# ishine/Prior-DiffuSE

Measured on AMD Instinct MI355X. Metric: enhanced-audio sec/sec (RTF), 6-step fast sampling, B=32, higher is better.
Workload: dtype f16x2; 1 GPU; B=32 x 4 s 16 kHz utterances per GPU, [B,2,401,161] spectrograms, GCRN prior + DiffUNet1 6-step sampling, STFT..ISTFT, seeded random weights; global_batch=32, frames=401, parallelism=batch-shard x1, graph=True, streams_per_gpu=1, batches_in_flight=3

## Files before the change

### __graft_entry__.py

```python
import importlib
import os
import subprocess
import sys

ROOT = os.path.dirname(os.path.abspath(__file__))
PKG = os.path.join(ROOT, "prior-diffuse_amd")
CSRC = os.path.join(PKG, "csrc")
SOURCES = ["gconv.hip", "gconv2.hip", "gconv3.hip", "gconv4.hip", "misc.hip", "lstm.hip", "lstmp.hip", "aia.hip", "tcm.hip", "tcm2.hip", "bglu.hip", "gru3.hip", "dense.hip", "metrics.hip", "stoi.hip", "resample.hip", "wavout.hip", "range.hip", "valid.hip", "objective.hip", "ensemble.hip", "window.hip", "capi.hip"]
LIB = os.path.join(PKG, "libpdse.so")


HASHFILE = LIB + ".srchash"


def _source_hash():
    import hashlib

    h = hashlib.sha256()
    included = sorted(f for f in os.listdir(CSRC) if f.endswith((".h", ".inc")))
    deps = [os.path.join(CSRC, s) for s in SOURCES + included] + [os.path.join(ROOT, "include", "pdse.h")]
    for d in deps:
        with open(d, "rb") as f:
            h.update(os.path.basename(d).encode() + b"\0" + f.read())
    return h.hexdigest()


def _stale():
    if not (os.path.exists(LIB) and os.path.exists(HASHFILE)):
        return True
    with open(HASHFILE) as f:
        return f.read().strip() != _source_hash()


def build(force=False):
    import torch

    import fcntl

    with open(os.path.join(PKG, ".build.lock"), "w") as lock:
        fcntl.flock(lock, fcntl.LOCK_EX)
        if force or _stale():
# ... 65 lines not shown
```

### include/pdse.h

```cpp
#ifndef PDSE_H
#define PDSE_H
#include <stdint.h>

#ifdef __cplusplus
extern "C" {
#endif

#define PDSE_ABI_VERSION 9

typedef void* pdse_stream_t;

enum pdse_act { PDSE_ACT_NONE = 0, PDSE_ACT_PRELU = 1, PDSE_ACT_ELU = 2, PDSE_ACT_SIGMOID = 3 };

enum pdse_epi {
  PDSE_EPI_LINEAR = 0,
  PDSE_EPI_GLU = 1,
  PDSE_EPI_BIGLU = 2
};

typedef struct pdse_src {
  const float* ptr;
  int64_t sb, sc, st, sf;
  int32_t C;
  int32_t act;
// ... 27 lines not shown
  int32_t act;
  float act_slope;
  int32_t C2;
  const float* post_scale;
  const float* post_shift;
  const float* wlc;
  const float* wrc;
  const float* blc;
  const float* brc;
  const float* wc2;
  const float* bc2;
  const float* resid;
  float* out;
  int64_t out_sb, out_sc_hi, out_sc_lo, out_st, out_sf, out_off;
  int32_t out_cr;
  int32_t B, Tout, Fout;
  int32_t korder;
  int32_t ksteps1;
  const float* w2;
  const float* w3;
  int32_t p1mask;
  int32_t Fout1;
  const float* nx_w;
  const float* nx_bias[3];
  const float* nx_add[3];
  float* nx_out[3];
  int64_t nx_bias_sb[3];
  int64_t nx_sb[3], nx_sc[3], nx_st[3], nx_sf[3], nx_off[3];
  int32_t nx_n, nx_keep, nx_row0;
  int32_t wexp;
  const float* bias0_t0;
  const float* bias1_t0;
  int32_t tap_dt[12], tap_df[12];
  int32_t flat, pad_;
} pdse_gconv_desc;

typedef struct pdse_time_desc {
  const float* t;
  const float* table;
  const float* p1T;
  const float* b1;
  const float* p2T;
  const float* b2;
  const float* wfT;
  const float* bf;
  float* out;
  float* temb;
  int32_t B, NF, max_steps, pad_;
} pdse_time_desc;

enum pdse_ew_op {
  PDSE_EW_DIV = 0,
  PDSE_EW_UPDATE = 1,
  PDSE_EW_UPDATE_FINAL = 2,
  PDSE_EW_COPY = 3,
  PDSE_EW_ADD_MUL = 4
};
typedef struct pdse_ew_desc {
  const float* a;
  const float* b;
  const float* c;
  float* out;
  int64_t n;
  float s0, s1, s2;
  int32_t op;
} pdse_ew_desc;

// ... 634 lines not shown
```

### prior-diffuse_amd/_lib.py

```python
import contextlib
import ctypes as C
import os

_HERE = os.path.dirname(os.path.abspath(__file__))
LIB_PATH = os.environ.get("PDSE_LIB") or os.path.join(_HERE, "libpdse.so")

ABI_VERSION = 9

ACT_NONE, ACT_PRELU, ACT_ELU, ACT_SIGMOID = 0, 1, 2, 3
EPI_LINEAR, EPI_GLU, EPI_BIGLU = 0, 1, 2
EW_DIV, EW_UPDATE, EW_UPDATE_FINAL, EW_COPY, EW_ADD_MUL = 0, 1, 2, 3, 4
(OP_GCONV, OP_TIME, OP_EW, OP_COMPAND, OP_WAVPREP, OP_OLA, OP_SIGMA, OP_LN, OP_LSTM,
 OP_ROWLN, OP_CHLN, OP_ATTN, OP_GRU, OP_GNCOMB, OP_AHAM, OP_QSAMPLE, OP_TRANSPOSE, OP_TCM, OP_CRM, OP_GCRNLAST,
 OP_MASKLOSS, OP_GLSTM, OP_TCM2, OP_BGLU, OP_PLANES, OP_GLSTMP, OP_TCM2S, OP_DENSE, OP_ROWLNB, OP_METRICS, OP_RESAMPLE, OP_RANGE) = range(32)
MASKLOSS_BLOCKS = 32
SPECLOSS_BLOCKS = 32

ENSEMBLE_BLOCKS = 32
ENSEMBLE_MAX = 16
_fp = C.c_void_p
_i32, _i64, _f32 = C.c_int32, C.c_int64, C.c_float


class Src(C.Structure):
    _fields_ = [("ptr", _fp), ("sb", _i64), ("sc", _i64), ("st", _i64), ("sf", _i64),
                ("C", _i32), ("act", _i32), ("blk", _i32), ("pad_", _i32)]


class GconvDesc(C.Structure):
    _fields_ = [
        ("in0", Src), ("in1", Src),
        ("Tin", _i32), ("Fin", _i32),
        ("padrow", _fp), ("padrow_sb", _i64),
        ("taps", _fp), ("ntaps", _i32), ("sf_in", _i32),
        ("xf_scale0", _fp), ("xf_shift0", _fp), ("xf_scale1", _fp), ("xf_shift1", _fp),
        ("xf_slope0", _f32), ("xf_slope1", _f32), ("xf_mode", _i32), ("cin1", _i32),
        ("w0", _fp), ("w1", _fp), ("ksteps", _i32), ("Cout", _i32),
        ("bias0", _fp), ("bias1", _fp), ("bias0_sb", _i64), ("bias1_sb", _i64),
        ("epi", _i32), ("act", _i32), ("act_slope", _f32), ("C2", _i32),
        ("post_scale", _fp), ("post_shift", _fp),
        ("wlc", _fp), ("wrc", _fp), ("blc", _fp), ("brc", _fp), ("wc2", _fp), ("bc2", _fp),
        ("resid", _fp), ("out", _fp),
        ("out_sb", _i64), ("out_sc_hi", _i64), ("out_sc_lo", _i64), ("out_st", _i64),
        ("out_sf", _i64), ("out_off", _i64),
        ("out_cr", _i32), ("B", _i32), ("Tout", _i32), ("Fout", _i32),
        ("korder", _i32), ("ksteps1", _i32), ("w2", _fp), ("w3", _fp), ("p1mask", _i32), ("Fout1", _i32),
        ("nx_w", _fp), ("nx_bias", _fp * 3), ("nx_add", _fp * 3), ("nx_out", _fp * 3), ("nx_bias_sb", _i64 * 3),
        ("nx_sb", _i64 * 3), ("nx_sc", _i64 * 3), ("nx_st", _i64 * 3), ("nx_sf", _i64 * 3), ("nx_off", _i64 * 3),
        ("nx_n", _i32), ("nx_keep", _i32), ("nx_row0", _i32), ("wexp", _i32),
        ("bias0_t0", _fp), ("bias1_t0", _fp),
        ("tap_dt", _i32 * 12), ("tap_df", _i32 * 12), ("flat", _i32), ("pad_", _i32),
    ]


class TimeDesc(C.Structure):
    _fields_ = [("t", _fp), ("table", _fp), ("p1T", _fp), ("b1", _fp), ("p2T", _fp), ("b2", _fp),
                ("wfT", _fp), ("bf", _fp), ("out", _fp), ("temb", _fp),
                ("B", _i32), ("NF", _i32), ("max_steps", _i32), ("pad_", _i32)]


class EwDesc(C.Structure):
    _fields_ = [("a", _fp), ("b", _fp), ("c", _fp), ("out", _fp), ("n", _i64),
                ("s0", _f32), ("s1", _f32), ("s2", _f32), ("op", _i32)]


class CompandDesc(C.Structure):
    _fields_ = [("in_", _fp), ("out", _fp), ("plane", _i64), ("B", _i32), ("mode", _i32),
                ("out_sb", _i64), ("out_sc", _i64), ("out_st", _i64), ("F", _i32), ("pad_", _i32)]


COMPAND_SQRT, COMPAND_SQUARE, COMPAND_MAG, COMPAND_COPY, COMPAND_POW03, COMPAND_POW103, COMPAND_LOG1X, COMPAND_EXPM1 = range(8)
FEAT_TYPES = ("sqrt", "normal", "cubic", "log_1x", "none")
COMPRESS_MODE = {"sqrt": COMPAND_SQRT, "normal": COMPAND_MAG, "cubic": COMPAND_POW03, "log_1x": COMPAND_LOG1X, "none": None}
DECOMPRESS_MODE = {"sqrt": COMPAND_SQUARE, "normal": COMPAND_COPY, "cubic": COMPAND_POW103, "log_1x": COMPAND_EXPM1,
                   "none": COMPAND_COPY}


def feat_type_of(value):
    if value not in FEAT_TYPES:
        raise ValueError("feat_type %r: must be one of 'sqrt', 'normal', 'cubic', 'log_1x', 'none'" % (value,))
    return value


def members_arg(members):
# ... 521 lines not shown
```

### prior-diffuse_amd/csrc/capi.hip

```cpp
#include <hip/hip_runtime.h>
#include <stdint.h>
#include <stdio.h>
#include <string.h>

#include <new>
#include <string>
#include <vector>

#include "pdse.h"
#include "pdse_internal.h"

static thread_local std::string g_err;

void pdse_set_error(const char* msg) { g_err = msg ? msg : "unknown error"; }

int pdse_check_hip(hipError_t e, const char* what) {
  if (e == hipSuccess) return 0;
  g_err = std::string(what) + ": " + hipGetErrorString(e);
  return 1;
}

int pdse_check_launch(const char* what) { return pdse_check_hip(hipGetLastError(), what); }

int pdse_lds_attr(const void* fn, unsigned long long* mask, const char* what) {
// ... 45 lines not shown
  explicit device_guard(const pdse_plan* p) {
    if (!p || p->device < 0) return;
    if (hipGetDevice(&prev) != hipSuccess) prev = -1;
    if (prev != p->device) ok = !pdse_check_hip(hipSetDevice(p->device), "set device");
    else prev = -1;
  }
  ~device_guard() {
    if (prev >= 0) (void)hipSetDevice(prev);
  }
};

static int op_size(int kind) {
  switch (kind) {
#define X(KIND, stem, entry) case PDSE_OP_##KIND: return (int)sizeof(pdse_##stem##_desc);
    PDSE_OPS(X)
#undef X
    default: return -1;
  }
}

static int launch_op(const pdse_op& op, hipStream_t s) {
  switch (op.kind) {
#define X(KIND, stem, entry) case PDSE_OP_##KIND: return pdse_##stem##_launch(&op.d.stem, s);
    PDSE_OPS(X)
#undef X
    default: pdse_set_error("plan: unknown op kind"); return 1;
  }
}

static bool names_odd_phase(const pdse_op& op) {
  return op.kind == PDSE_OP_GCONV && op.d.gconv.korder == 5 && op.d.gconv.p1mask != 0 && op.d.gconv.w2 == nullptr;
}

static int check_follows(const pdse_plan* p, const pdse_op& op) {
  if (p->ops.empty() || !names_odd_phase(p->ops.back())) return 0;
  if (op.kind != PDSE_OP_GCONV) {
    pdse_set_error("plan: the operator behind a gconv that names its odd phase (p1mask, korder 5) must be that phase");
    return 1;
  }
  return pdse_gconv_pair_check(&p->ops.back().d.gconv, &op.d.gconv);
}

static int launch_at(const pdse_plan* p, const int i, const int end, hipStream_t s, int* n) {
  const pdse_op& op = p->ops[i];
  *n = 1;
  if (names_odd_phase(op) && i + 1 < end) {
    *n = 2;
    return pdse_gconv4_pair_launch(&op.d.gconv, &p->ops[i + 1].d.gconv, s);
  }
  return launch_op(op, s);
}

template <typename D>
static int validate_desc(const D*) { return 0; }
static int validate_desc(const pdse_range_desc* d) { return pdse_range_validate(d); }

extern "C" {

int pdse_abi_version(void) { return PDSE_ABI_VERSION; }
const char* pdse_last_error(void) { return g_err.c_str(); }
int pdse_desc_size(int op_kind) { return op_size(op_kind); }

#define X(KIND, stem, entry) \
  int entry(const pdse_##stem##_desc* d, pdse_stream_t s) { return validate_desc(d) ? 1 : pdse_##stem##_launch(d, (hipStream_t)s); }
PDSE_OPS(X)
#undef X

int pdse_wav_encode(const float* x, const int32_t* n_in_host, const int32_t* n_keep_host, const int32_t* n_in, const int32_t* n_keep,
                    const double* taps, uint8_t* out, int32_t* clipped, int64_t stride, int32_t B, int32_t Lmax, int32_t up, int32_t down,
                    int32_t half, int32_t fmt, int32_t width, int32_t ch, pdse_stream_t s) {
  return pdse_wavout_launch(x, n_in_host, n_keep_host, n_in, n_keep, taps, out, clipped, stride, B, Lmax, up, down, half, fmt, width, ch,
                            (hipStream_t)s);
}

int pdse_wav_encode_channels(const float* x, const int32_t* n_in_host, const int32_t* n_keep_host, const int32_t* n_in,
                             const int32_t* n_keep, const double* taps, uint8_t* out, int32_t* clipped, int64_t stride, int32_t B,
                             int32_t Lmax, int32_t up, int32_t down, int32_t half, int32_t fmt, int32_t width, int32_t ch, pdse_stream_t s) {
  return pdse_wavch_launch(x, n_in_host, n_keep_host, n_in, n_keep, taps, out, clipped, stride, B, Lmax, up, down, half, fmt, width, ch,
                           (hipStream_t)s);
}

// ... 441 lines not shown
```

### prior-diffuse_amd/csrc/gconv.hip

```cpp
#include <hip/hip_runtime.h>
#include <stdint.h>

#include "pdse.h"
#include "pdse_internal.h"

#include "gconv_common.h"

template <int EPI, int MT, bool CIN1>
__global__ __launch_bounds__(256) void gconv_kernel(const pdse_gconv_desc d) {
  constexpr bool DUAL = (EPI != PDSE_EPI_LINEAR);
  const int lane = threadIdx.x & 63, wave = threadIdx.x >> 6;
  const int col = lane & 31, h = lane >> 5;
  const int b = blockIdx.y;
  const int P = d.Tout * d.Fout;
  const int p = (blockIdx.x * 4 + wave) * 32 + col;
  const bool pvalid = p < P;
  const int t = pvalid ? p / d.Fout : 0;
  const int j = pvalid ? p - t * d.Fout : 0;
  const int mtiles = (d.Cout + 31) >> 5;
  const int mt0 = blockIdx.z * MT;

  f32x16 acc0[MT], acc1[DUAL ? MT : 1];
#pragma unroll
  for (int m = 0; m < MT; ++m) {
// ... 73 lines not shown
      float v = 0.f;
      if (pvalid && tap < d.ntaps) {
        const int tin = t + d.taps[2 * tap], fin = j * d.sf_in + d.taps[2 * tap + 1];
        if (tin >= 0 && tin < d.Tin && fin >= 0 && fin < d.Fin) {
          v = base[(int64_t)tin * S.st + (int64_t)fin * S.sf];
          if (S.act) v = act_f(v, S.act, 0.f);
        }
      }
#pragma unroll
      for (int m = 0; m < MT; ++m) {
        if (mt0 + m < mtiles) {
          const float a0 = wp0[((size_t)m * ksteps + ks) * 64];
          acc0[m] = __builtin_amdgcn_mfma_f32_32x32x2f32(a0, v, acc0[m], 0, 0, 0);
          if (DUAL) {
            const float a1 = wp1[((size_t)m * ksteps + ks) * 64];
            acc1[m] = __builtin_amdgcn_mfma_f32_32x32x2f32(a1, v, acc1[m], 0, 0, 0);
          }
        }
      }
    }
  }

  gconv_epilogue<EPI, MT>(d, tail_from_desc(d), acc0, acc1, b, t, j, pvalid, lane, h, mt0, mtiles);
}

#define PDSE_REQUIRE(cond, msg)    \
  do {                             \
    if (!(cond)) {                 \
      pdse_set_error("gconv: " msg); \
      return 1;                    \
    }                              \
  } while (0)

static int gconv_launch(const pdse_gconv_desc* d, hipStream_t s, const bool dry) {
  PDSE_REQUIRE(d != nullptr, "null descriptor");
  PDSE_REQUIRE(!dry || d->korder == 5, "a phase pair is two korder 5 launches");
  PDSE_REQUIRE(d->in0.ptr && d->out && d->w0 && d->taps, "null pointer (in0/out/w0/taps)");
  PDSE_REQUIRE(d->B > 0 && d->B <= 65535 && d->Tout > 0 && d->Fout > 0, "bad output extents");
  PDSE_REQUIRE(d->Cout > 0 && d->ntaps > 0 && d->out_cr > 0, "bad Cout/ntaps/out_cr");
  PDSE_REQUIRE((int64_t)d->Tout * d->Fout < (1ll << 30), "too many positions per batch item");
  const int Cin = d->in0.C + d->in1.C;
  if (d->cin1) {
    PDSE_REQUIRE(Cin == 1 && d->in1.C == 0, "cin1 path needs exactly one input channel");
    PDSE_REQUIRE(d->ksteps == (d->ntaps + 1) / 2, "ksteps != ceil(ntaps/2)");
    PDSE_REQUIRE(d->xf_mode == 0 && d->padrow == nullptr, "cin1 path has no load transform / pad row");
  } else {
    PDSE_REQUIRE(Cin >= 2 && (d->in0.C % 2) == 0 && (d->in1.C % 2) == 0, "channel counts must be even");
    PDSE_REQUIRE(d->in1.C == 0 || d->in1.ptr, "in1 has channels but no pointer");
    if (d->korder == 0) PDSE_REQUIRE(d->ksteps == d->ntaps * (Cin / 2), "ksteps != ntaps*Cin/2");
    else PDSE_REQUIRE(d->ksteps >= d->ntaps * (Cin / 2), "ksteps < ntaps*Cin/2");
    PDSE_REQUIRE(d->korder < 3 || d->epi != PDSE_EPI_BIGLU, "korder 3 / 4 / 5 have LINEAR / GLU epilogues only");
  }
  PDSE_REQUIRE((d->in0.blk == 0 && d->in1.blk == 0) || d->korder == 3 || d->korder == 4 || d->korder == 5, "channel-blocked sources (pdse_src.blk) are read by the korder 3 kernel only");
  PDSE_REQUIRE(d->flat == 0 || d->korder == 3 || d->korder == 5, "the flat form (pdse_gconv_desc.flat) is one of the korder 3 / 5 kernel");
  if (d->xf_mode) {
    PDSE_REQUIRE(d->xf_scale0 && d->xf_shift0, "xf_mode set without scale/shift");
    PDSE_REQUIRE(d->xf_mode != 2 || (d->xf_scale1 && d->xf_shift1), "xf_mode 2 without second set");
  }
  PDSE_REQUIRE((d->post_scale == nullptr) == (d->post_shift == nullptr), "post_scale/post_shift must come together");
  {
    auto al16 = [](const void* p) { return (reinterpret_cast<uintptr_t>(p) & 15) == 0; };
    PDSE_REQUIRE(al16(d->bias0) && al16(d->bias1) && al16(d->post_scale) && al16(d->post_shift) && al16(d->blc) &&
                     al16(d->brc) && al16(d->bc2) && al16(d->bias0_t0) && al16(d->bias1_t0),
                 "per-channel operands (biases, folded BatchNorm) must be 16-byte aligned");
    PDSE_REQUIRE((d->bias0_sb & 3) == 0 && (d->bias1_sb & 3) == 0, "bias batch strides must be multiples of 4 floats");
  }
  PDSE_REQUIRE(d->resid == nullptr || d->act == PDSE_ACT_NONE, "a residual input excludes an activation (x + f(..) is the last op)");
  if (d->nx_n != 0) {
    PDSE_REQUIRE(d->nx_n > 0 && d->nx_n <= 3 && d->nx_w, "nx: 1..3 chained tiles and their weights");
    PDSE_REQUIRE(d->epi == PDSE_EPI_BIGLU && (d->korder == 1 || d->korder == 2) && d->C2 == 64 && d->out_cr == 1,
                 "nx: chained 1x1 tiles need the pipelined BIGLU kernel with a 64-channel block output");
    for (int i = 0; i < d->nx_n; ++i) PDSE_REQUIRE(d->nx_bias[i] && d->nx_out[i], "nx: bias / output pointer missing");
    PDSE_REQUIRE(d->nx_row0 < d->nx_n, "nx_row0 out of range");
    PDSE_REQUIRE(d->w2 == nullptr || (d->nx_n == 1 && d->nx_keep == 0 && d->nx_row0 < 0),
                 "nx: a dual-phase launch chains one tile and does not keep its own output");
    PDSE_REQUIRE(d->nx_keep == 0 || d->out, "nx_keep without an output pointer");
  }
  PDSE_REQUIRE((d->bias0_t0 == nullptr) == (d->bias1_t0 == nullptr), "bias0_t0 / bias1_t0 must come together");
  PDSE_REQUIRE(d->bias0_t0 == nullptr || (d->nx_n > 0 && d->w2 == nullptr),
               "frame-0 biases are a feature of the chained single-phase BIGLU tail");
  if (d->korder == 1) {
    PDSE_REQUIRE(!d->cin1, "korder 1 needs Cin >= 2");
    return pdse_gconv2_launch(d, s);
  }
  if (d->korder >= 3 && d->korder <= 5) return dry ? 0 : pdse_gconv4_launch(d, s);
  if (d->korder == 2) {
    PDSE_REQUIRE(d->resid == nullptr, "BIGLU has no residual input");
    PDSE_REQUIRE(d->act == PDSE_ACT_NONE || d->act == PDSE_ACT_PRELU, "BIGLU stages end in PReLU or no activation");
    return pdse_gconv3_launch(d, s);
  }
  PDSE_REQUIRE(d->korder == 0, "unknown korder");
  const int mtiles = (d->Cout + 31) / 32;
  const int P = d->Tout * d->Fout;
  const int gx = ((P + 31) / 32 + 3) / 4;
  dim3 block(256);
  auto grid = [&](int mt) { return dim3(gx, d->B, (mtiles + mt - 1) / mt); };

#define LAUNCH(EPI, MT, C1)                                                          \
  hipLaunchKernelGGL((gconv_kernel<EPI, MT, C1>), grid(MT), block, 0, s, *d)

  switch (d->epi) {
    case PDSE_EPI_LINEAR: {
      if (d->cin1) {
        if (mtiles >= 4) LAUNCH(PDSE_EPI_LINEAR, 4, true);
        else if (mtiles >= 2) LAUNCH(PDSE_EPI_LINEAR, 2, true);
        else LAUNCH(PDSE_EPI_LINEAR, 1, true);
      } else {
        if (mtiles >= 4) LAUNCH(PDSE_EPI_LINEAR, 4, false);
        else if (mtiles >= 2) LAUNCH(PDSE_EPI_LINEAR, 2, false);
        else LAUNCH(PDSE_EPI_LINEAR, 1, false);
      }
      break;
    }
    case PDSE_EPI_GLU: {
      PDSE_REQUIRE(d->w1 != nullptr && !d->cin1, "GLU needs w1 and Cin >= 2");
      if (mtiles >= 4) LAUNCH(PDSE_EPI_GLU, 4, false);
      else if (mtiles >= 2) LAUNCH(PDSE_EPI_GLU, 2, false);
      else LAUNCH(PDSE_EPI_GLU, 1, false);
      break;
    }
    case PDSE_EPI_BIGLU: {
      PDSE_REQUIRE(d->w1 && !d->cin1 && d->Cout == 32, "BIGLU needs w1 and a 32-channel gate pair");
      PDSE_REQUIRE(d->bias0 && d->bias1 && d->wlc && d->wrc && d->blc && d->brc && d->wc2 && d->bc2,
                   "BIGLU chain pointers missing");
      PDSE_REQUIRE(d->C2 == 1 || (d->C2 > 0 && d->C2 % 32 == 0), "BIGLU C2 must be 1 or a multiple of 32");
      PDSE_REQUIRE(d->resid == nullptr, "BIGLU has no residual input");
      PDSE_REQUIRE(d->act == PDSE_ACT_NONE || d->act == PDSE_ACT_PRELU, "BIGLU stages end in PReLU or no activation");
      LAUNCH(PDSE_EPI_BIGLU, 1, false);
      break;
    }
    default:
      pdse_set_error("gconv: unknown epilogue");
      return 1;
  }
#undef LAUNCH
  return pdse_check_launch("gconv");
}

int pdse_gconv_launch(const pdse_gconv_desc* d, hipStream_t s) { return gconv_launch(d, s, false); }

int pdse_gconv_pair_check(const pdse_gconv_desc* d, const pdse_gconv_desc* e) {
  if (gconv_launch(d, nullptr, true) || gconv_launch(e, nullptr, true)) return 1;
  return pdse_gconv4_pair_check(d, e);
}
```

### prior-diffuse_amd/csrc/pdse_internal.h

```cpp
#ifndef PDSE_INTERNAL_H
#define PDSE_INTERNAL_H
#include <hip/hip_runtime.h>

#include "pdse.h"

void pdse_set_error(const char* msg);
int pdse_check_launch(const char* what);
int pdse_check_hip(hipError_t e, const char* what);
int pdse_lds_attr(const void* fn, unsigned long long* mask, const char* what);
#ifdef PDSE_DIAG
#define PDSE_DIAG_ENV(name) (getenv(name))
#else
#define PDSE_DIAG_ENV(name) ((const char*)nullptr)
#endif

#define PDSE_OPS(X)                                                                            \
  X(GCONV, gconv, pdse_gconv_f32)                                                              \
  X(TIME, time, pdse_time_embed_f32)                                                           \
  X(EW, ew, pdse_ew_f32)                                                                       \
  X(COMPAND, compand, pdse_compand_f32)                                                        \
  X(WAVPREP, wavprep, pdse_wavprep_f32)                                                        \
  X(OLA, ola, pdse_ola_f32)                                                                    \
  X(SIGMA, sigma, pdse_sigma_mask_f32)                                                         \
  X(LN, ln, pdse_layernorm_f32)                                                                \
// ... 1 lines not shown
  X(ROWLN, rowln, pdse_rowln_prelu_f32)                                                        \
  X(CHLN, chln, pdse_chln_f32)                                                                 \
  X(ATTN, attn, pdse_attention_f32)                                                            \
  X(GRU, gru, pdse_bigru_f32)                                                                  \
  X(GNCOMB, gncomb, pdse_gn_combine_f32)                                                       \
  X(AHAM, aham, pdse_aham_f32)                                                                 \
  X(QSAMPLE, qsample, pdse_qsample_f32)                                                        \
  X(TRANSPOSE, transpose, pdse_transpose_f32)                                                  \
  X(TCM, tcm, pdse_tcm_f32)                                                                    \
  X(CRM, crm, pdse_crm_f32)                                                                    \
  X(GCRNLAST, gcrnlast, pdse_gcrnlast_f32)                                                     \
  X(MASKLOSS, maskloss, pdse_masked_mse_f32)                                                   \
  X(GLSTM, glstm, pdse_glstm_f32)                                                              \
  X(TCM2, tcm2, pdse_tcm2_bf16x3)                                                              \
  X(BGLU, bglu, pdse_bglu_planes)                                                              \
  X(PLANES, planes, pdse_split_planes)                                                         \
  X(GLSTMP, glstmp, pdse_glstm_persistent_f32)                             \
  X(TCM2S, tcm2s, pdse_tcm2_stack_bf16x3)    \
  X(DENSE, dense, pdse_dense_layer_bf16x3)                                 \
  X(ROWLNB, rowlnb, pdse_rowln_blocked_f32)                                                    \
  X(METRICS, metrics, pdse_quality_metrics_f32)                          \
  X(RESAMPLE, resample, pdse_pcm_resample_f32)                          \
  X(RANGE, range, pdse_range_hist)

#define X(KIND, stem, entry) int pdse_##stem##_launch(const pdse_##stem##_desc* d, hipStream_t s);
PDSE_OPS(X)
#undef X
int pdse_gconv2_launch(const pdse_gconv_desc* d, hipStream_t s);
int pdse_gconv3_launch(const pdse_gconv_desc* d, hipStream_t s);
int pdse_gconv4_launch(const pdse_gconv_desc* d, hipStream_t s);
int pdse_gconv_pair_check(const pdse_gconv_desc* d, const pdse_gconv_desc* e);
int pdse_gconv4_pair_check(const pdse_gconv_desc* d, const pdse_gconv_desc* e);
int pdse_gconv4_pair_launch(const pdse_gconv_desc* d, const pdse_gconv_desc* e, hipStream_t s);
int pdse_stoi_launch(const pdse_metrics_desc* d, hipStream_t s);
int pdse_gru3_launch(const pdse_gru_desc* d, hipStream_t s);
int pdse_wavout_launch(const float* x, const int32_t* n_in_host, const int32_t* n_keep_host, const int32_t* n_in, const int32_t* n_keep,
                       const double* taps, uint8_t* out, int32_t* clipped, int64_t stride, int32_t B, int32_t Lmax, int32_t up,
                       int32_t down, int32_t half, int32_t fmt, int32_t width, int32_t ch, hipStream_t s);
int pdse_wavch_launch(const float* x, const int32_t* n_in_host, const int32_t* n_keep_host, const int32_t* n_in, const int32_t* n_keep,
                      const double* taps, uint8_t* out, int32_t* clipped, int64_t stride, int32_t B, int32_t Lmax, int32_t up,
                      int32_t down, int32_t half, int32_t fmt, int32_t width, int32_t ch, hipStream_t s);
int pdse_pair_prep_launch(const float* noisy, const float* clean, const int32_t* lens, float* noisy_pad, float* clean_pad, float* c,
                          int32_t B, int32_t L, int32_t pad, int32_t reflect_own, hipStream_t s);
int pdse_spec_losses_launch(const float* esti, const float* label, const int32_t* frames_host, const int32_t* frames, double* partial,
                            double* per_utt, float* loss, int32_t B, int32_t T, int32_t F, hipStream_t s);
int pdse_spec_frames_launch(const float* spec, const double* basis, float* frames, int32_t B, int32_t T, int32_t F, hipStream_t s);
int pdse_spec_frames_mode_launch(const float* spec, const double* basis, float* frames, int32_t B, int32_t T, int32_t F, int32_t mode,
                                 hipStream_t s);
int pdse_objective_noise_launch(const float* label, const float* init, const float* noise, const int32_t* t, const float* a_tab,
                                const float* s_tab, float* noisy, float* target, float* maxbuf, int32_t B, int32_t T, int32_t F,
                                int32_t mode, int32_t sigma, hipStream_t s);
int pdse_sigma_loss_launch(const float* predicted, const float* target, const float* init, const float* maxbuf,
                           const int32_t* frames_host, const int32_t* frames, double* partial, double* per_utt, float* loss, int32_t B,
                           int32_t T, int32_t F, hipStream_t s);
int pdse_ensemble_stats_launch(const float* members, float* mean, float* spread, const int32_t* frames_host, const int32_t* frames,
                               double* partial, double* per_utt, double* per_member, int32_t K, int32_t B, int32_t T, int32_t F,
                               hipStream_t s);
int pdse_window_gather_launch(const float* whole, float* win, int32_t B, int32_t C, int32_t T, int32_t F, int32_t W, int32_t a,
                              hipStream_t s);
int pdse_window_scatter_launch(const float* win, float* whole, int32_t B, int32_t C, int32_t T, int32_t F, int32_t W, int32_t a,
                               int32_t keep_lo, int32_t keep_hi, hipStream_t s);
int pdse_range_validate(const pdse_range_desc* d);
#endif
```

### prior-diffuse_amd/nets.py

```python
import ctypes as C

import numpy as np
import torch

from . import _lib as L
from . import packing as P

F0 = 161
BIG = 1 << 30

TAG_NONE, TAG_EPS_BLOCK, TAG_EPS_CONV1, TAG_TCM, TAG_PRIOR, TAG_LSTM, TAG_SIGNAL, TAG_EW = range(8)


class WeightBank:

    def __init__(self):
        self.items = {}
        self.keep = []
        self.owners = []

    def token(self, obj):
        if obj is None:
            return None
        for i, o in enumerate(self.owners):
# ... 126 lines not shown

    def audited(self):
        out, seen = [], set()
        for addr, kind, box, suffix in self._audit_ops.values():
            hit = next(((n, t) for n, t in self._audit_names.values()
                        if t.data_ptr() <= addr < t.data_ptr() + t.numel() * t.element_size()), None)
            if hit is None:
                raise RuntimeError("range audit: the f16x2 operand at 0x%x lies in no buffer the builder named (PlanBase.named)" % addr)
            name, t = hit
            key = (name + suffix, kind)
            if key in seen:
                continue
            seen.add(key)
            out.append((name + suffix, t, kind, P.F16_ACT_EXP if kind == L.RANGE_F32 else 0,
                        None if box is None else dict(box, off=(addr - t.data_ptr()) // 2)))
        return out

    def finish(self):
        if self.plan is not None:
            self.plan.keep(self.ctx.keep, self.ctx.bank)

    carries_state = False

    def receptive_field(self):
        return None

    def src(self, t, C_, sb, sc, st, sf, off=0, act=L.ACT_NONE, blk=0):
        return L.Src(Ctx.ptr(t, off), sb, sc, st, sf, C_, act, blk, 0)

    def gconv(self, *, in0, in1=None, Tin, Fin, taps, sf_in, W, Cout, bias0=None, bias0_sb=0,
              bias1=None, bias1_sb=0, epi=L.EPI_LINEAR, act=L.ACT_NONE, act_slope=0.0,
              padrow=None, padrow_sb=0, padrow_off=0, cin1=False, resid=None, out,
              out_strides, out_off=0, out_cr=1, B, Tout, Fout, tag=TAG_NONE, bias0_off=0, phase1=None, nx=None,
              bias1_off=0, bias_t0=None, label="gconv", s3=False, s3g=False, has_xf=False, flat=False):
        ctx = self.ctx
        d = L.GconvDesc()
        d.in0 = in0
        d.in1 = in1 if in1 is not None else L.Src(0, 0, 0, 0, 0, 0, 0)
        d.Tin, d.Fin = Tin, Fin
        d.padrow, d.padrow_sb = Ctx.ptr(padrow, padrow_off), padrow_sb
        ttaps = tuple((int(a), int(b)) for a, b in taps)
        tkey = ("taps", ttaps)
        tp = ctx.bank.items.get(tkey)
        if tp is None:
            ctx._banking += 1
            tp = ctx.bank.items[tkey] = self._up(P.taps_array(ttaps))
            ctx._banking -= 1
        d.taps, d.ntaps, d.sf_in = tp.data_ptr(), len(ttaps), sf_in
        for i, (dt_, df_) in enumerate(ttaps[:12]):
            d.tap_dt[i], d.tap_df[i] = dt_, df_
        d.cin1 = 1 if cin1 else 0
        c0, c1 = d.in0.C, d.in1.C
        pipelined_ok = padrow is None and not self.force_generic
        s3 = bool(s3) and pipelined_ok and epi == L.EPI_BIGLU and (
            ((c0, c1) == (32, 0) and len(ttaps) in (4, 6)) or ((c0, c1, len(ttaps)) == (2, 2, 10) and phase1 is None))
        s3g = (bool(s3g) and not s3 and pipelined_ok and epi in (L.EPI_LINEAR, L.EPI_GLU) and not cin1 and not has_xf
               and c0 > 0 and c0 % 16 == 0 and c1 % 16 == 0 and len(ttaps) <= 12)
        site = "%s:%d:%d:%d:%d:%d:%d:%d:%d" % (label, epi, len(ttaps), c0, c1, Cout, pipelined_ok, s3, s3g)
        if s3g:
            pack = lambda: P.gconv_gemm_fields(W(), len(ttaps), c0, c1, self.gemm_planes)
        elif s3:
            pack = lambda: P.gconv_s3_fields(W(), len(ttaps), c0 + c1)
        else:
            pack = lambda: P.gconv_fields(W(), len(ttaps), c0, c1, epi, cin1, pipelined_ok)
        self.apply(d, self.fields(site, pack))
        d.Cout = Cout
        if bias0 is not None:
            d.bias0 = Ctx.ptr(bias0, bias0_off)
        if bias1 is not None:
            d.bias1 = Ctx.ptr(bias1, bias1_off)
        d.bias0_sb, d.bias1_sb = bias0_sb, bias1_sb
        if bias_t0 is not None:
            d.bias0_t0, d.bias1_t0 = Ctx.ptr(bias_t0[0], bias_t0[1]), Ctx.ptr(bias_t0[0], bias_t0[2])
        d.epi, d.act, d.act_slope = epi, act, float(act_slope)
        if phase1 is not None and d.korder in (1, 2):
            d.p1mask, d.Fout1 = phase1["mask"], phase1["Fout1"]
        elif phase1 is not None and d.korder == 5 and epi == L.EPI_GLU:
            d.p1mask, d.Fout1 = phase1["mask"], phase1["Fout1"]
        if nx is not None:
            tiles = nx["tiles"]
            d.nx_n, d.nx_keep, d.nx_row0 = len(tiles), 1 if nx.get("keep") else 0, nx.get("row0", -1)
            for i, tl in enumerate(tiles):
                if tl.get("bias") is not None:
                    d.nx_bias[i] = Ctx.ptr(tl["bias"], tl.get("bias_off", 0))
                d.nx_bias_sb[i] = tl.get("bias_sb", 0)
                d.nx_out[i] = Ctx.ptr(tl["out"])
                d.nx_sb[i], d.nx_sc[i], d.nx_st[i], d.nx_sf[i] = tl["strides"]
                d.nx_off[i] = tl.get("off", 0)
                d.nx_add[i] = Ctx.ptr(tl.get("add"))
        d.resid = Ctx.ptr(resid)
        d.out = Ctx.ptr(out)
        d.out_sb, d.out_sc_hi, d.out_sc_lo, d.out_st, d.out_sf = out_strides
        d.out_off, d.out_cr = out_off, out_cr
        d.B, d.Tout, d.Fout = B, Tout, Fout
        d.flat = 1 if flat and s3g and d.korder in (3, 5) else 0
        self.add(d, tag)
        return d


def nchw(C_, T, F):
    return C_ * T * F, T * F, F, 1


def nchw_out(C_, T, F):
    return C_ * T * F, T * F, 0, F, 1


def nc8(C_, T, F):
    return C_ * T * F, T * F * 8, F * 8, 8


def nc8_out(C_, T, F):
    return C_ * T * F, T * F * 8, 1, F * 8, 8


class EpsNetPlan(PlanBase):

    ENC_F = [161, 79, 39, 19, 9, 4]
    fused_tcm = True
    chain_conv1 = True
    compose_stage1 = True
    split_bf16 = True
    split_tcm = True
    plane_h = True
    tcm_stack = True
    parity_planes = True
    planes = 2
    TCM_F16 = True
# ... 626 lines not shown
                else:
                    in1 = self.src(skip, 64, *nchw(64, T, self.ENC_F[k]))
                p = "%s.de%d.0" % (de, k)
                if k > 1:
                    o, ooff = self.dec[n & 1], 0
                    fn = lambda Fo: nchw_out(64, T, Fo)
                    bn, pr = "%s.de%d.2" % (de, k), "%s.de%d.3.weight" % (de, k)
                else:
                    o, ooff = out, di * T * F0
                    fn = lambda Fo: nchw_out(2, T, Fo)
                    bn, pr = None, None
                nx = None
                if chained and k > 1:
                    Fo = 2 * (Fin - 1) + 3
                    wn = lambda de=de, k=k: self.w("%s.de%d.0.conv1.weight" % (de, k - 1))[:, :, 0, 0].T[:, :64]
                    nx = dict(keep=False, row0=-1, tiles=[dict(wfn=wn, bias=self.zero32, out=Hn, add=self.Pskip[di][k - 1],
                                                                strides=(32 * T * Fo, T * Fo, Fo, 2))])
                Fin = self._biconvtransglu(step, 5 + 5 * di + n, p, k, in0, in1, Fin, o, fn, bn, pr, out_off=ooff, H=Hc,
                                           do_conv1=(k == 5 or not chained), nx=nx)
                if chained:
                    Hc, Hn = Hn, Hc
                in0 = self.src(o, 64, *nchw(64, T, Fin))
        return out


class GcrnPlan(PlanBase):
    fused_last = True
    fused_glstm = True
    split_bf16 = True
    gemm_planes = 2
    block8 = True
    fuse_phases = True
    flat_proj = True
    persist_lstm = True
    chunk_proj = True
    CHUNK_TC = 32
    PERSIST_MAX_B = 4
    ENC_C = [2, 16, 32, 64, 128, 256]
    ENC_F = [161, 80, 39, 19, 9, 4]
    carries_state = True

    def receptive_field(self):
        return 0, 0

    def __init__(self, ctx, sd, B, T, plan=None, split_bf16=None, exclusive=False, planes=None, carry_state=False):
        self.carry_state = bool(carry_state)
        if self.carry_state:
            exclusive = False
            if not self.fused_glstm or self.force_generic:
                raise ValueError("carry_state needs the wavefront form of the grouped LSTM (csrc/lstm.hip: glstm_wave_kernel)")
        if split_bf16 is not None:
            self.split_bf16 = bool(split_bf16)
        if planes is not None:
            if planes not in (1, 2, 3) or (planes in (1, 2) and not self.split_bf16):
                raise ValueError("planes is 3 (bf16x3), 2 (f16x2) or 1 (bf16 mode); the one- and two-plane forms run on the GEMM kernels (split_bf16)")
            self.gemm_planes = int(planes)
        self.persist = bool(self.persist_lstm and self.fused_glstm and exclusive and B <= self.PERSIST_MAX_B and not self.force_generic)
        self.exclusive = bool(exclusive)
        self.chunk = bool(self.chunk_proj and self.fused_glstm and not exclusive and not self.persist and not self.force_generic
                          and T >= 2 * self.CHUNK_TC)
        super().__init__(ctx, plan, ns=(ctx.bank.token(sd), self.fused_last, self.fused_glstm, self.split_bf16, self.block8, self.persist,
                                        self.gemm_planes))
        self.sd, self.B, self.T = sd, B, T
        a = ctx.alloc
        self.Bp = Bp = (B + 31) // 32 * 32
        self.status = None
# ... 102 lines not shown
        d = L.LnDesc()
        d.blk = blk
        d.in_, d.out = self.y.data_ptr(), out_t.data_ptr()
        d.gamma = self.upw(name + ".g", lambda: self.w(name + ".weight")).data_ptr()
        d.beta = self.upw(name + ".b", lambda: self.w(name + ".bias")).data_ptr()
        d.osb, d.os_hi, d.os_lo, d.os_t = osb, os_hi, os_lo, os_t
        d.B, d.T, d.N, d.r, d.eps = self.B, self.T, 1024, r, 1e-5
        self.add(d, TAG_PRIOR)

    def build(self, x=None, out=None):
        B, T, Bp = self.B, self.T, self.Bp
        x = self.x if x is None else x
        out = self.out if out is None else out
        blk = self.split_bf16 and not self.force_generic and self.block8

        def lay(k_is_blocked, C_, Fq):
            if k_is_blocked:
                return nc8(C_, T, Fq), nc8_out(C_, T, Fq), 8
            return nchw(C_, T, Fq), nchw_out(C_, T, Fq), 1

        src = self.src(x, 2, *nchw(2, T, F0))
        e_lay = [lay(blk and k >= 2, self.ENC_C[k], self.ENC_F[k]) for k in range(1, 6)]
        for k in range(1, 6):
            ci, co, Fin, Fout = self.ENC_C[k - 1], self.ENC_C[k], self.ENC_F[k - 1], self.ENC_F[k]
            kk, taps = P.conv_taps(1, 3, 0)
            p = "conv%d" % k
            ist, ost_, ocr = e_lay[k - 1]
            self.gconv(in0=src, Tin=T, Fin=Fin, taps=taps, sf_in=2, Cout=co, epi=L.EPI_GLU, act=L.ACT_ELU,
                       W=lambda p=p, k=k, kk=kk: dict(wk0=P.conv_kmat(self.sd[p + ".conv1.weight"], kk),
                                                      wk1=P.conv_kmat(self.sd[p + ".conv2.weight"], kk),
                                                      bias0=self.w(p + ".conv1.bias"), bias1=self.w(p + ".conv2.bias"),
                                                      post=P.bn_fold(self.sd, "bn%d" % k)),
                       out=self.e[k - 1], out_strides=ost_, out_cr=ocr, B=B, Tout=T, Fout=Fout, tag=TAG_PRIOR, label=p,
                       s3g=self.split_bf16)
            src = self.src(self.e[k - 1], co, *ist, blk=8 if ocr == 8 else 0)

        def proj1(g):
            wk = lambda Wih: np.concatenate([Wih[:, f::4].T for f in range(4)], axis=0)
            s = self.src(self.e[4], 128, *e_lay[4][0], off=128 * g * T * 4, blk=8 if blk else 0)
            return s, T, 4, [(0, f) for f in range(4)], wk, T, 1, 2048 * Bp, 0

        if self.persist:
            self._glstm_persistent(proj1)
        elif self.fused_glstm and not self.force_generic:
            self._glstm_wavefront(proj1)
        else:
            self._lstm_layer("lstm_list1", proj1, y_su=2, y_sg=1)
            self._ln("glstm.ln1", self.yn, 1024 * T, T, 0, 1, 1)

            def proj2(g):
                s = self.src(self.yn, 512, 1024 * T, T, 0, 1, off=512 * g * T)
                return s, 1, T, [(0, 0)], (lambda Wih: Wih.T), 1, T, 0, 2048 * Bp

            self._lstm_layer("lstm_list2", proj2, y_su=1, y_sg=512)
        if blk:
            self._ln("glstm.ln2", self.glstm, 256 * T * 4, T * 4 * 8, 8, 4 * 8, 4, blk=8)
        else:
            self._ln("glstm.ln2", self.glstm, 256 * T * 4, T * 4, 1, 4, 4)

        dec = [(5, 512, 128), (4, 256, 64), (3, 128, 32), (2, 64, 16), (1, 32, 1)]
        for br in (1, 2):
            in0 = self.src(self.glstm, 256, *(nc8(256, T, 4) if blk else nchw(256, T, 4)), blk=8 if blk else 0)
            in1 = self.src(self.e[4], 256, *e_lay[4][0], blk=8 if blk else 0)
            Fin = 4
            for n, (k, ci, co) in enumerate(dec):
                p = "conv%d_t_%d" % (k, br)
                Fout = 2 * (Fin - 1) + 3 + (1 if k == 2 else 0)
# ... 496 lines not shown
```

Before: 10010 audio_s/s.

## Fuse the first two GCRN encoder conv layers into one kernel

Adds a dedicated kernel that computes GCRN encoder layer 1 (2->16 channels, GLU+ELU, scalar FMA) into an LDS tile and feeds it straight into layer 2 (16->32 channels, split-plane MMA) within the same block. The plan marks layer 1 with an enc flag and the dispatcher launches both as one pair. This removes one launch and the re-read of layer 1's output from global memory by layer 2, though layer 1's output is still written out. It relies on strict shape and stride checks and hardcodes the 161/80/39-bin geometry.

Result: no change. 10050 audio_s/s, median of 6 (+0.4%).

```diff
diff --git a/__graft_entry__.py b/__graft_entry__.py
--- a/__graft_entry__.py
+++ b/__graft_entry__.py
@@ -6,7 +6,7 @@
 ROOT = os.path.dirname(os.path.abspath(__file__))
 PKG = os.path.join(ROOT, "prior-diffuse_amd")
 CSRC = os.path.join(PKG, "csrc")
-SOURCES = ["gconv.hip", "gconv2.hip", "gconv3.hip", "gconv4.hip", "misc.hip", "lstm.hip", "lstmp.hip", "aia.hip", "tcm.hip", "tcm2.hip", "bglu.hip", "gru3.hip", "dense.hip", "metrics.hip", "stoi.hip", "resample.hip", "wavout.hip", "range.hip", "valid.hip", "objective.hip", "ensemble.hip", "window.hip", "capi.hip"]
+SOURCES = ["gconv.hip", "gconv2.hip", "gconv3.hip", "gconv4.hip", "gcrnenc.hip", "misc.hip", "lstm.hip", "lstmp.hip", "aia.hip", "tcm.hip", "tcm2.hip", "bglu.hip", "gru3.hip", "dense.hip", "metrics.hip", "stoi.hip", "resample.hip", "wavout.hip", "range.hip", "valid.hip", "objective.hip", "ensemble.hip", "window.hip", "capi.hip"]
 LIB = os.path.join(PKG, "libpdse.so")
 
 
diff --git a/include/pdse.h b/include/pdse.h
--- a/include/pdse.h
+++ b/include/pdse.h
@@ -83,7 +83,8 @@
   const float* bias0_t0;
   const float* bias1_t0;
   int32_t tap_dt[12], tap_df[12];
-  int32_t flat, pad_;
+  int32_t flat;
+  int32_t enc;
 } pdse_gconv_desc;
 
 typedef struct pdse_time_desc {
diff --git a/prior-diffuse_amd/_lib.py b/prior-diffuse_amd/_lib.py
--- a/prior-diffuse_amd/_lib.py
+++ b/prior-diffuse_amd/_lib.py
@@ -49,7 +49,7 @@
         ("nx_sb", _i64 * 3), ("nx_sc", _i64 * 3), ("nx_st", _i64 * 3), ("nx_sf", _i64 * 3), ("nx_off", _i64 * 3),
         ("nx_n", _i32), ("nx_keep", _i32), ("nx_row0", _i32), ("wexp", _i32),
         ("bias0_t0", _fp), ("bias1_t0", _fp),
-        ("tap_dt", _i32 * 12), ("tap_df", _i32 * 12), ("flat", _i32), ("pad_", _i32),
+        ("tap_dt", _i32 * 12), ("tap_df", _i32 * 12), ("flat", _i32), ("enc", _i32),
     ]
 
 
diff --git a/prior-diffuse_amd/csrc/capi.hip b/prior-diffuse_amd/csrc/capi.hip
--- a/prior-diffuse_amd/csrc/capi.hip
+++ b/prior-diffuse_amd/csrc/capi.hip
@@ -101,7 +101,16 @@
   return op.kind == PDSE_OP_GCONV && op.d.gconv.korder == 5 && op.d.gconv.p1mask != 0 && op.d.gconv.w2 == nullptr;
 }
 
+static bool names_enc_layer2(const pdse_op& op) { return op.kind == PDSE_OP_GCONV && op.d.gconv.enc != 0; }
+
 static int check_follows(const pdse_plan* p, const pdse_op& op) {
+  if (!p->ops.empty() && names_enc_layer2(p->ops.back())) {
+    if (op.kind != PDSE_OP_GCONV) {
+      pdse_set_error("plan: the operator behind a gconv marked enc must be the second encoder layer");
+      return 1;
+    }
+    return pdse_gconv_enc_check(&p->ops.back().d.gconv, &op.d.gconv);
+  }
   if (p->ops.empty() || !names_odd_phase(p->ops.back())) return 0;
   if (op.kind != PDSE_OP_GCONV) {
     pdse_set_error("plan: the operator behind a gconv that names its odd phase (p1mask, korder 5) must be that phase");
@@ -116,6 +125,10 @@
   if (names_odd_phase(op) && i + 1 < end) {
     *n = 2;
     return pdse_gconv4_pair_launch(&op.d.gconv, &p->ops[i + 1].d.gconv, s);
+  }
+  if (names_enc_layer2(op) && i + 1 < end) {
+    *n = 2;
+    return pdse_gcrnenc_launch(&op.d.gconv, &p->ops[i + 1].d.gconv, s);
   }
   return launch_op(op, s);
 }
diff --git a/prior-diffuse_amd/csrc/gconv.hip b/prior-diffuse_amd/csrc/gconv.hip
--- a/prior-diffuse_amd/csrc/gconv.hip
+++ b/prior-diffuse_amd/csrc/gconv.hip
@@ -129,9 +129,11 @@
     }                              \
   } while (0)
 
-static int gconv_launch(const pdse_gconv_desc* d, hipStream_t s, const bool dry) {
+static int gconv_launch(const pdse_gconv_desc* d, hipStream_t s, const int dry) {
   PDSE_REQUIRE(d != nullptr, "null descriptor");
-  PDSE_REQUIRE(!dry || d->korder == 5, "a phase pair is two korder 5 launches");
+  PDSE_REQUIRE(dry != 1 || d->korder == 5, "a phase pair is two korder 5 launches");
+  PDSE_REQUIRE(dry != 2 || d->korder == 1 || d->korder == 5, "the fused encoder layers are a korder 1 and a korder 5 launch");
+  PDSE_REQUIRE(d->enc == 0 || d->enc == 1, "enc (pdse_gconv_desc.enc) is 0 or 1");
   PDSE_REQUIRE(d->in0.ptr && d->out && d->w0 && d->taps, "null pointer (in0/out/w0/taps)");
   PDSE_REQUIRE(d->B > 0 && d->B <= 65535 && d->Tout > 0 && d->Fout > 0, "bad output extents");
   PDSE_REQUIRE(d->Cout > 0 && d->ntaps > 0 && d->out_cr > 0, "bad Cout/ntaps/out_cr");
@@ -178,7 +180,7 @@
                "frame-0 biases are a feature of the chained single-phase BIGLU tail");
   if (d->korder == 1) {
     PDSE_REQUIRE(!d->cin1, "korder 1 needs Cin >= 2");
-    return pdse_gconv2_launch(d, s);
+    return dry ? 0 : pdse_gconv2_launch(d, s);
   }
   if (d->korder >= 3 && d->korder <= 5) return dry ? 0 : pdse_gconv4_launch(d, s);
   if (d->korder == 2) {
@@ -234,9 +236,14 @@
   return pdse_check_launch("gconv");
 }
 
-int pdse_gconv_launch(const pdse_gconv_desc* d, hipStream_t s) { return gconv_launch(d, s, false); }
+int pdse_gconv_launch(const pdse_gconv_desc* d, hipStream_t s) { return gconv_launch(d, s, 0); }
 
 int pdse_gconv_pair_check(const pdse_gconv_desc* d, const pdse_gconv_desc* e) {
-  if (gconv_launch(d, nullptr, true) || gconv_launch(e, nullptr, true)) return 1;
+  if (gconv_launch(d, nullptr, 1) || gconv_launch(e, nullptr, 1)) return 1;
   return pdse_gconv4_pair_check(d, e);
 }
+
+int pdse_gconv_enc_check(const pdse_gconv_desc* d, const pdse_gconv_desc* e) {
+  if (gconv_launch(d, nullptr, 2) || gconv_launch(e, nullptr, 2)) return 1;
+  return pdse_gcrnenc_check(d, e);
+}
diff --git a/prior-diffuse_amd/csrc/gcrnenc.hip b/prior-diffuse_amd/csrc/gcrnenc.hip
--- /dev/null
+++ b/prior-diffuse_amd/csrc/gcrnenc.hip
@@ -0,0 +1,213 @@
+#include <hip/hip_runtime.h>
+#include <stdint.h>
+
+#include "pdse.h"
+#include "pdse_internal.h"
+
+#include "gconv_common.h"
+
+#define ENC_R 8
+#define ENC_NT 320
+#define ENC_P 80
+#define ENC_F0 161
+#define ENC_F1 80
+#define ENC_F2 39
+#define ENC_COLS (ENC_R * ENC_F2)
+#define ENC_CT ((ENC_COLS + 31) / 32)
+
+template <bool CR1>
+__global__ __launch_bounds__(ENC_NT, 3) void gcrn_enc_kernel(const pdse_gconv_desc d, const pdse_gconv_desc e, const int tpw) {
+  __shared__ __attribute__((aligned(16))) float tile[ENC_R * 16 * ENC_P];
+  __shared__ uint4 wfrag[2 * 3 * 2 * 64];
+  __shared__ __attribute__((aligned(16))) float w1tab[16 * 16];
+  const int tid = threadIdx.x;
+  const int lane = tid & 63, wave = __builtin_amdgcn_readfirstlane(tid >> 6);
+  const int col = lane & 31, h = lane >> 5;
+  const int T = d.Tout;
+  const long long N = (long long)d.B * T;
+  const int ntiles = (int)((N + ENC_R - 1) / ENC_R);
+
+  for (int i = tid; i < 2 * 384; i += ENC_NT)
+    wfrag[i] = reinterpret_cast<const uint4*>(i < 384 ? e.w0 : e.w1)[i < 384 ? i : i - 384];
+  if (tid < 256) {
+    const int c = tid >> 4, k = tid & 15;
+    float v;
+    if (k < 12) {
+      const int kk = k < 6 ? k : k - 6, tap = kk >> 1, ci = kk & 1;
+      v = (k < 6 ? d.w0 : d.w1)[(32 * ci + c) * 4 + tap];
+    } else if (k == 12) v = d.bias0 ? d.bias0[c] : 0.f;
+    else if (k == 13) v = d.bias1 ? d.bias1[c] : 0.f;
+    else if (k == 14) v = d.post_scale ? d.post_scale[c] : 1.f;
+    else v = d.post_scale ? d.post_shift[c] : 0.f;
+    w1tab[tid] = v;
+  }
+
+  const int hh = tid >= 160, rem = tid - 160 * hh;
+  const int r1 = rem / 20, q1 = rem - 20 * r1;
+  auto load_x = [&](const int tl, float (&x)[2][9]) {
+    const long long n = (long long)tl * ENC_R + r1;
+    const bool ok = tl < ntiles && n < N;
+    const int b = ok ? (int)(n / T) : 0, t = ok ? (int)(n - (long long)b * T) : 0;
+    const float* p = d.in0.ptr + ((int64_t)b * d.in0.sb + (int64_t)t * d.in0.st + 8 * q1);
+#pragma unroll
+    for (int ci = 0; ci < 2; ++ci)
+#pragma unroll
+      for (int k = 0; k < 9; ++k) x[ci][k] = ok ? p[(int64_t)ci * d.in0.sc + k] : 0.f;
+  };
+
+  const int tile0 = blockIdx.x * tpw;
+  float xc[2][9], xn[2][9];
+  load_x(tile0, xc);
+  __syncthreads();
+
+  const float us = pow2i(-(PDSE_F16_ACT_EXP + e.wexp));
+#pragma unroll 1
+  for (int it = 0; it < tpw; ++it) {
+    const int tl = tile0 + it;
+    if (tl >= ntiles) break;
+    load_x(it + 1 < tpw ? tl + 1 : ntiles, xn);
+
+    {
+      const long long n = (long long)tl * ENC_R + r1;
+      const bool ok = n < N;
+      const int b = ok ? (int)(n / T) : 0, t = ok ? (int)(n - (long long)b * T) : 0;
+      float* const po = d.out + ((int64_t)b * d.out_sb + (int64_t)t * d.out_st + d.out_off + 4 * q1);
+      float* const pl = tile + (r1 * 16 + 8 * hh) * ENC_P + 4 * q1;
+#pragma unroll 1
+      for (int cc = 0; cc < 8; ++cc) {
+        const int c = 8 * hh + cc;
+        const float4 wa = *reinterpret_cast<const float4*>(w1tab + 16 * c), wb = *reinterpret_cast<const float4*>(w1tab + 16 * c + 4),
+                     wc = *reinterpret_cast<const float4*>(w1tab + 16 * c + 8), wd = *reinterpret_cast<const float4*>(w1tab + 16 * c + 12);
+        const float wm[6] = {wa.x, wa.y, wa.z, wa.w, wb.x, wb.y}, wg[6] = {wb.z, wb.w, wc.x, wc.y, wc.z, wc.w};
+        f32x4 v4;
+#pragma unroll
+        for (int i = 0; i < 4; ++i) {
+          float m = 0.f, g = 0.f;
+#pragma unroll
+          for (int tap = 0; tap < 3; ++tap)
+#pragma unroll
+            for (int ci = 0; ci < 2; ++ci) {
+              m = fmaf(wm[2 * tap + ci], xc[ci][2 * i + tap], m);
+              g = fmaf(wg[2 * tap + ci], xc[ci][2 * i + tap], g);
+            }
+          float y = (m + wd.x) * sigmoid_f(g + wd.y);
+          y = y * wd.z + wd.w;
+          v4[i] = act_c<PDSE_ACT_ELU>(y, 0.f);
+        }
+        if (ok) *reinterpret_cast<f32x4*>(po + (int64_t)c * d.out_sc_hi) = v4;
+        *reinterpret_cast<f32x4*>(pl + cc * ENC_P) = v4;
+      }
+    }
+    __syncthreads();
+
+#pragma unroll 1
+    for (int ct = wave; ct < ENC_CT; ct += 5) {
+      const int p = ct * 32 + col;
+      const int r = p / ENC_F2, j = p - r * ENC_F2;
+      const long long n = (long long)tl * ENC_R + r;
+      const bool pvalid = p < ENC_COLS && n < N;
+      const int b = pvalid ? (int)(n / T) : 0, t = pvalid ? (int)(n - (long long)b * T) : 0;
+      const int rr = pvalid ? r : 0, jj = pvalid ? j : 0;
+      f32x16 acc0, acc1;
+#pragma unroll
+      for (int q = 0; q < 16; ++q) acc0[q] = acc1[q] = 0.f;
+#pragma unroll
+      for (int tap = 0; tap < 3; ++tap) {
+        const float* src = tile + (rr * 16 + 8 * h) * ENC_P + 2 * jj + tap;
+        float x[8];
+#pragma unroll
+        for (int q = 0; q < 8; ++q) x[q] = pvalid ? src[q * ENC_P] : 0.f;
+        uint4 bp[2];
+        split_planes<2>(x, bp, pow2i(PDSE_F16_ACT_EXP));
+        const uint4 a0[2] = {wfrag[(tap * 2) * 64 + lane], wfrag[(tap * 2 + 1) * 64 + lane]};
+        const uint4 a1[2] = {wfrag[(6 + tap * 2) * 64 + lane], wfrag[(6 + tap * 2 + 1) * 64 + lane]};
+        acc0 = plane_mma<2>(a0, bp, acc0);
+        acc1 = plane_mma<2>(a1, bp, acc1);
+      }
+#pragma unroll
+      for (int q = 0; q < 16; ++q) {
+        acc0[q] *= us;
+        acc1[q] *= us;
+      }
+      if (pvalid) {
+        float* const ob = e.out + ((int64_t)b * e.out_sb + (int64_t)t * e.out_st + (int64_t)j * e.out_sf + e.out_off);
+        const int64_t cstep = e.out_sc_hi;
+        f32x16 y = acc0, g = acc1;
+        if (e.bias0) y += ld16(e.bias0 + 4 * h);
+        if (e.bias1) g += ld16(e.bias1 + 4 * h);
+#pragma unroll
+        for (int q = 0; q < 16; ++q) y[q] *= sigmoid_f(g[q]);
+        if (e.post_scale) y = y * ld16(e.post_scale + 4 * h) + ld16(e.post_shift + 4 * h);
+        if constexpr (CR1) {
+          float* const po = ob + (int64_t)(4 * h) * cstep;
+#pragma unroll
+          for (int q = 0; q < 16; ++q) po[(int64_t)PDSE_KR(q) * cstep] = act_c<PDSE_ACT_ELU>(y[q], 0.f);
+        } else {
+          float* const po = ob + 4 * h;
+#pragma unroll
+          for (int q = 0; q < 4; ++q) {
+            f32x4 v4;
+#pragma unroll
+            for (int i = 0; i < 4; ++i) v4[i] = act_c<PDSE_ACT_ELU>(y[4 * q + i], 0.f);
+            *reinterpret_cast<f32x4*>(po + (int64_t)q * cstep) = v4;
+          }
+        }
+      }
+    }
+    __syncthreads();
+#pragma unroll
+    for (int ci = 0; ci < 2; ++ci)
+#pragma unroll
+      for (int k = 0; k < 9; ++k) xc[ci][k] = xn[ci][k];
+  }
+}
+
+#define ENC_REQUIRE(cond, msg)                  \
+  do {                                          \
+    if (!(cond)) {                              \
+      pdse_set_error("gcrn enc: " msg);         \
+      return 1;                                 \
+    }                                           \
+  } while (0)
+
+int pdse_gcrnenc_check(const pdse_gconv_desc* d, const pdse_gconv_desc* e) {
+  auto taps3 = [](const pdse_gconv_desc* x) {
+    return x->ntaps == 3 && x->tap_dt[0] == 0 && x->tap_dt[1] == 0 && x->tap_dt[2] == 0 && x->tap_df[0] == 0 && x->tap_df[1] == 1 &&
+           x->tap_df[2] == 2 && x->sf_in == 2;
+  };
+  auto plain = [](const pdse_gconv_desc* x) {
+    return x->epi == PDSE_EPI_GLU && x->act == PDSE_ACT_ELU && x->in1.C == 0 && x->in0.act == PDSE_ACT_NONE && x->in0.blk == 0 &&
+           x->in0.sf == 1 && x->padrow == nullptr && x->xf_mode == 0 && x->cin1 == 0 && x->resid == nullptr && x->w1 != nullptr &&
+           x->w2 == nullptr && x->nx_n == 0 && x->p1mask == 0 && x->flat == 0 && x->Tin == x->Tout && x->bias0_sb == 0 &&
+           x->bias1_sb == 0;
+  };
+  ENC_REQUIRE(d->enc == 1, "the mark (pdse_gconv_desc.enc) is 1");
+  ENC_REQUIRE(d->korder == 1 && plain(d) && taps3(d) && d->in0.C == 2 && d->Cout == 16 && d->Fin == ENC_F0 && d->Fout == ENC_F1,
+              "the marked launch is the first encoder layer: korder 1, GLU + ELU, one plain source of 2 channels and 161 bins, "
+              "taps (0,0) (0,1) (0,2) at stride 2, 16 channels of 80 bins");
+  ENC_REQUIRE(d->out_cr == 1 && d->out_sf == 1 && !((d->out_sb | d->out_sc_hi | d->out_st | d->out_off) & 3) &&
+                  (reinterpret_cast<uintptr_t>(d->out) & 15) == 0,
+              "the first layer's output has contiguous bins and 16-byte aligned rows (out_cr 1, out_sf 1, strides in multiples of 4)");
+  ENC_REQUIRE(e->enc == 0 && e->korder == 5 && plain(e) && taps3(e) && e->in0.C == 16 && e->Cout == 32 && e->Fin == ENC_F1 &&
+                  e->Fout == ENC_F2 && e->B == d->B && e->Tout == d->Tout,
+              "the operator behind the mark is the second encoder layer: korder 5, GLU + ELU, one plain source of 16 channels and "
+              "80 bins, the same taps, batch and frames, 32 channels of 39 bins");
+  ENC_REQUIRE(e->out_cr == 1 || (e->out_cr == 8 && e->out_sc_lo == 1 && !((e->out_sb | e->out_sc_hi | e->out_st | e->out_sf | e->out_off) & 3) &&
+                                 (reinterpret_cast<uintptr_t>(e->out) & 15) == 0),
+              "the second layer's output is plain (out_cr 1) or channel-blocked (out_cr 8, out_sc_lo 1, strides in multiples of 4, "
+              "a 16-byte aligned base)");
+  ENC_REQUIRE(e->in0.ptr == d->out + d->out_off && e->in0.sb == d->out_sb && e->in0.sc == d->out_sc_hi && e->in0.st == d->out_st,
+              "the second layer reads what the first writes (source pointer and strides)");
+  ENC_REQUIRE((long long)d->B * d->Tout <= (1ll << 30), "too many rows");
+  return 0;
+}
+
+int pdse_gcrnenc_launch(const pdse_gconv_desc* d, const pdse_gconv_desc* e, hipStream_t s) {
+  const long long N = (long long)d->B * d->Tout;
+  const int ntiles = (int)((N + ENC_R - 1) / ENC_R);
+  const int tpw = ntiles >= 1024 ? 2 : 1;
+  const dim3 grid((ntiles + tpw - 1) / tpw), block(ENC_NT);
+  if (e->out_cr == 1) hipLaunchKernelGGL(gcrn_enc_kernel<true>, grid, block, 0, s, *d, *e, tpw);
+  else hipLaunchKernelGGL(gcrn_enc_kernel<false>, grid, block, 0, s, *d, *e, tpw);
+  return pdse_check_launch("gcrn enc");
+}
diff --git a/prior-diffuse_amd/csrc/pdse_internal.h b/prior-diffuse_amd/csrc/pdse_internal.h
--- a/prior-diffuse_amd/csrc/pdse_internal.h
+++ b/prior-diffuse_amd/csrc/pdse_internal.h
@@ -57,6 +57,9 @@
 int pdse_gconv_pair_check(const pdse_gconv_desc* d, const pdse_gconv_desc* e);
 int pdse_gconv4_pair_check(const pdse_gconv_desc* d, const pdse_gconv_desc* e);
 int pdse_gconv4_pair_launch(const pdse_gconv_desc* d, const pdse_gconv_desc* e, hipStream_t s);
+int pdse_gconv_enc_check(const pdse_gconv_desc* d, const pdse_gconv_desc* e);
+int pdse_gcrnenc_check(const pdse_gconv_desc* d, const pdse_gconv_desc* e);
+int pdse_gcrnenc_launch(const pdse_gconv_desc* d, const pdse_gconv_desc* e, hipStream_t s);
 int pdse_stoi_launch(const pdse_metrics_desc* d, hipStream_t s);
 int pdse_gru3_launch(const pdse_gru_desc* d, hipStream_t s);
 int pdse_wavout_launch(const float* x, const int32_t* n_in_host, const int32_t* n_keep_host, const int32_t* n_in, const int32_t* n_keep,
diff --git a/prior-diffuse_amd/nets.py b/prior-diffuse_amd/nets.py
--- a/prior-diffuse_amd/nets.py
+++ b/prior-diffuse_amd/nets.py
@@ -182,7 +182,7 @@
               bias1=None, bias1_sb=0, epi=L.EPI_LINEAR, act=L.ACT_NONE, act_slope=0.0,
               padrow=None, padrow_sb=0, padrow_off=0, cin1=False, resid=None, out,
               out_strides, out_off=0, out_cr=1, B, Tout, Fout, tag=TAG_NONE, bias0_off=0, phase1=None, nx=None,
-              bias1_off=0, bias_t0=None, label="gconv", s3=False, s3g=False, has_xf=False, flat=False):
+              bias1_off=0, bias_t0=None, label="gconv", s3=False, s3g=False, has_xf=False, flat=False, enc=False):
         ctx = self.ctx
         d = L.GconvDesc()
         d.in0 = in0
@@ -244,6 +244,7 @@
         d.out_off, d.out_cr = out_off, out_cr
         d.B, d.Tout, d.Fout = B, Tout, Fout
         d.flat = 1 if flat and s3g and d.korder in (3, 5) else 0
+        d.enc = 1 if enc and d.korder == 1 else 0
         self.add(d, tag)
         return d
 
@@ -936,6 +937,7 @@
     block8 = True
     fuse_phases = True
     flat_proj = True
+    fuse_enc = True
     persist_lstm = True
     chunk_proj = True
     CHUNK_TC = 32
@@ -1104,7 +1106,8 @@
                                                       bias0=self.w(p + ".conv1.bias"), bias1=self.w(p + ".conv2.bias"),
                                                       post=P.bn_fold(self.sd, "bn%d" % k)),
                        out=self.e[k - 1], out_strides=ost_, out_cr=ocr, B=B, Tout=T, Fout=Fout, tag=TAG_PRIOR, label=p,
-                       s3g=self.split_bf16)
+                       s3g=self.split_bf16,
+                       enc=k == 1 and self.fuse_enc and self.split_bf16 and self.gemm_planes == 2 and not self.force_generic)
             src = self.src(self.e[k - 1], co, *ist, blk=8 if ocr == 8 else 0)
 
         def proj1(g):
```
